# MP-Gadget/shenqi

Hardware: AMD Instinct MI355X
Metric: particle-steps/sec (grav+PM+SPH) at 256^3; rms force error vs ref (higher is better)
Workload: dtype f64

## Files before the change

__graft_entry__.py:

```python
import os
import subprocess
import sys

ROOT = os.path.dirname(os.path.abspath(__file__))


def build():
    env = dict(os.environ)
    env.setdefault("HIPCC", "/opt/rocm/bin/hipcc")
    subprocess.check_call(["make", "-C", ROOT, "-j4", "all"], env=env)
    if ROOT not in sys.path:
        sys.path.insert(0, ROOT)
    import shenqi_amd


def smoke():
    if ROOT not in sys.path:
        sys.path.insert(0, ROOT)
    sys.path.insert(0, os.path.join(ROOT, "tests"))
    import numpy as np
    import shenqi_amd as sq
    import common as cm
    import orc

    n = 16**3
    pos = cm.random_positions(orc.boost_mt19937_uniform(0, 3 * n), n)
    pman = cm.make_partmanager(pos)
    pm = dict(Asmth=1.5, Nmesh=48, G=cm.G)
    cm.reference_treepar(ErrTolForceAcc=0.002, MaxBHOpeningAngle=0.9, TreeUseBH=0)
    sq.gravshort_set_softenings(cm.BOX / np.cbrt(n))
    gp_rel = sq.make_grav_params(cm.BOX, 1.5, 48, cm.G, cm.RHO0)
    with sq.Context(0) as ctx:
        sq.gravpm_force(ctx, pm, pman)
        tree = sq.force_tree_full(pman)
        cm.reference_treepar(ErrTolForceAcc=0.002, MaxBHOpeningAngle=0.9)
        sq.gravshort_set_softenings(cm.BOX / np.cbrt(n))
        sq.grav_short_tree(ctx, None, pm, tree, None, cm.RHO0)
        gpm = pman.Base["GravPM"].copy()
        seed = pman.Base["FullTreeGravAccel"].copy()
        st = sq.grav_short_tree(ctx, None, pm, tree, None, cm.RHO0)
        acc = pman.Base["FullTreeGravAccel"].copy()
        import ctypes as C
        from shenqi_amd import capi
        tb = sq.tree_build_device(ctx, cm.BOX)
        capi.check(capi.hip.shq_grav_short_run(ctx.h, C.byref(gp_rel), None, 0, 1, sq.WALK_EXACT))
        nint_dev = np.zeros(n, dtype=np.int64)
        capi.check(capi.hip.shq_grav_short_download(ctx.h, None, None, capi.ptr(nint_dev), None))
        pmp = sq.PMParams(48, 0, cm.BOX, 1.5, cm.G)
        capi.check(capi.hip.shq_treepm_step(ctx.h, C.byref(pmp), C.byref(gp_rel), 1, sq.WALK_EXACT))
        fused = C.c_int(0)
        capi.check(capi.hip.shq_treepm_last_fused(ctx.h, C.byref(fused)))
        gpm_step = np.zeros((n, 3)); acc_step = np.zeros((n, 3)); nint_step = np.zeros(n, dtype=np.int64)
        capi.check(capi.hip.shq_pm_download(ctx.h, capi.ptr(gpm_step), None))
        capi.check(capi.hip.shq_grav_short_download(ctx.h, capi.ptr(acc_step), None, capi.ptr(nint_step), None))
    mass = pman.Base["Mass"]
    ogpm, _, _, _ = orc.pm_force(pos, mass, 48, cm.BOX, 1.5, cm.G)
    cm.reference_treepar(ErrTolForceAcc=0.002, MaxBHOpeningAngle=0.9, TreeUseBH=0)
    gp = sq.make_grav_params(cm.BOX, 1.5, 48, cm.G, cm.RHO0)
    oacc, opot, onint = orc.grav_walk(tree.Nodes_base, tree.firstnode, pos, mass,
                                      np.linalg.norm(seed + gpm, axis=1) / cm.G, gp)
    oacc *= cm.G
    e_pm = np.abs(gpm - ogpm).max() / np.abs(ogpm).max()
    e_tree = np.abs(acc - oacc).max() / np.abs(oacc).max()
    assert e_pm < 1e-9, e_pm
    assert e_tree < 1e-10, e_tree
    assert st.ninteractions == int(onint.sum())
    assert tb.numnodes > 0 and np.array_equal(nint_dev, onint), "walk on the device-built tree differs from the oracle"
    assert fused.value == 0, "shq_treepm_step took the fused-readout route, which is off by default"
    assert np.abs(gpm_step - ogpm).max() / np.abs(ogpm).max() < 1e-9
    oacc2, _, onint2 = orc.grav_walk(tree.Nodes_base, tree.firstnode, pos, mass, np.linalg.norm(acc + gpm_step, axis=1) / cm.G, gp)
    assert np.array_equal(nint_step, onint2), "shq_treepm_step: interaction counts differ from the oracle"
    assert np.abs(acc_step - oacc2 * cm.G).max() / np.abs(oacc2).max() / cm.G < 1e-10
    ng = 10**3
    gpos = cm.BOX * orc.boost_mt19937_uniform(7, 3 * ng).reshape(ng, 3)
    gman, SphP, BhP = cm.make_gas(gpos, np.full(ng, cm.BOX / 10))
    BhP = np.zeros(2, dtype=sq.BH_SLOT_DTYPE)
    sq.set_densitypar(DensityResolutionEta=1.0, MaxNumNgbDeviation=0.5, DensityKernelType=1, BlackHoleNgbFactor=2.0, MinGasHsml=0.006)
    ost = orc.SphState(gman.Base, SphP, BhP)
    onodes, ofirst, ofather = orc.tree_build(gpos, gman.Base["Mass"], cm.BOX)
    rc, oevp, _, oniter, _ = orc.density(onodes, ofirst, ofather, ost, cm.density_params(DoEgyDensity=1))
    assert rc == 0
    orc.update_hmax(onodes, ofirst, ost)
    orc.hydro(onodes, ofirst, ost, cm.hydro_params(), oevp)
    with sq.Context(0) as ctx:
        gtree = sq.force_tree_rebuild_mask(gman, sq.GASMASK)
        evp, dst = sq.density(ctx, None, 1, 1, 0, None, gtree, gman, SphP, BhP)
        sq.force_tree_update_hmax(gtree, gman)
        sq.set_hydropar(1, 100.0, 0.75)
        sq.hydro_force(ctx, None, 0.1, cm.HUBBLE, evp, None, gtree, gman, SphP)
    e_rho = np.abs(SphP["Density"] / ost.density - 1).max()
    e_hyd = np.abs(SphP["HydroAccel"] - ost.hydroaccel).max() / np.abs(ost.hydroaccel).max()
    assert dst.niterations == oniter and e_rho < 1e-10 and e_hyd < 1e-9, (dst.niterations, oniter, e_rho, e_hyd)
    print(f"smoke ok: PM rel err {e_pm:.2e}, tree rel err {e_tree:.2e}, SPH density rel err {e_rho:.2e}, hydro rel err {e_hyd:.2e}, "
          f"{st.ninteractions / n:.1f} interactions/target, walk {st.kernel_ms:.3f} ms, "
          f"device tree build {tb.numnodes} nodes in {tb.build_ms:.3f} ms")


if __name__ == "__main__":
    build()
    if len(sys.argv) > 1 and sys.argv[1] == "smoke":
        smoke()
```

shenqi_amd/csrc/common.hpp:

```cpp
#ifndef SHQ_COMMON_HPP
#define SHQ_COMMON_HPP

#include <hip/hip_runtime.h>
#include <hipfft/hipfft.h>
#include <stdint.h>
#include <stdio.h>
#include <string>
#include <vector>
#include "../../include/shenqi_hip.h"
#include "yields_math.hpp"
#include "cooling_math.hpp"

void shq_set_error(const char *fmt, ...);

#define SHQ_HIP(call)                                                                          \
    do {                                                                                       \
        hipError_t e_ = (call);                                                                \
        if(e_ != hipSuccess) {                                                                 \
            shq_set_error("%s:%d: %s failed: %s", __FILE__, __LINE__, #call, hipGetErrorString(e_)); \
            return (e_ == hipErrorOutOfMemory) ? SHQ_ERR_NOMEM : SHQ_ERR_DEVICE;               \
        }                                                                                      \
    } while(0)

#define SHQ_CHECK(cond, code, ...)                                                             \
// ... 30 lines not shown
            ptr = nullptr;
            return SHQ_ERR_NOMEM;
        }
        cap = n;
        return SHQ_OK;
    }
    void release()
    {
        if(ptr)
            (void) hipFree(ptr);
        ptr = nullptr;
        cap = 0;
    }
};

template <typename T> struct PinBuf {
    T *ptr = nullptr;
    size_t cap = 0;
    int reserve(size_t n)
    {
        if(n <= cap)
            return SHQ_OK;
        if(ptr)
            (void) hipHostFree(ptr);
        ptr = nullptr;
        cap = 0;
        hipError_t e = hipHostMalloc((void **) &ptr, n * sizeof(T), hipHostMallocDefault);
        if(e != hipSuccess) {
            shq_set_error("hipHostMalloc of %zu bytes failed: %s", n * sizeof(T), hipGetErrorString(e));
            ptr = nullptr;
            return SHQ_ERR_NOMEM;
        }
        cap = n;
        return SHQ_OK;
    }
    void release()
    {
        if(ptr)
            (void) hipHostFree(ptr);
        ptr = nullptr;
        cap = 0;
    }
};

struct NodeA { double cofm[3]; double mass; };
struct NodeB { double center[3]; double len; };
struct NodeC { int32_t sibling; int32_t child; int32_t type; int32_t count; };
struct NodeH { double hmax; };
struct alignas(128) NodeG {
    double cofm[3], mass;
    double center[3], len;
    int32_t sibling, child, type, count;
    double bhlim;
    double mlen2;
    double inside;
    double rcut2;
    double wraplim;
    double rcuthl;
};
static_assert(sizeof(NodeG) == 128, "NodeG must be one 128-byte line");

struct alignas(32) TopNodeG {
    double cofm[3], mass;
    double center[3], len;
    double hmax;
    int32_t sibling, child;
    int32_t kind;
    int32_t leaf;
    double pad;
};
static_assert(sizeof(TopNodeG) == 96, "TopNodeG layout");

struct GravStatsDev {
    unsigned long long ninteractions;
    unsigned long long nvisited;
    unsigned long long nwave_applies;
    unsigned long long nwave_node_applies;
    unsigned long long nnode_interactions;
    long long min_int;
    long long max_int;
    unsigned long long hist_visit[8], hist_node[8], hist_leaf[8];
    unsigned long long lonely[4];
};

__device__ __forceinline__ unsigned long long shq_ballot(bool p) { return __builtin_amdgcn_ballot_w64(p); }

__device__ __forceinline__ unsigned xcd_block(unsigned b, unsigned nb, unsigned K = 16)
{
    if(K == 0)
        return b;
    const unsigned super = b / (8u * K);
    if((super + 1u) * 8u * K > nb)
        return b;
    const unsigned within = b - super * 8u * K;
    return super * 8u * K + (within & 7u) * K + (within >> 3);
}

#define SHQ_NTIMERS 20
enum { SHQ_T_PM0 = 8 , SHQ_T_SPH = 14, SHQ_T_TREE = 16, SHQ_T_WALK = SHQ_NTIMERS - 1 };

struct TreeBuildBufs {
    DevBuf<unsigned long long> keys[2], okeys[2], packed[2], counters;
    DevBuf<int> state;
    DevBuf<int32_t> idx[2], order[2], rank, frontier[2], bounds;
    DevBuf<int32_t> lo, hi, parent, sibling, firstchild, nchild, level;
    DevBuf<int32_t> top;
    DevBuf<unsigned long long> path;
    DevBuf<int4> geo_child[2];
    DevBuf<int2> geo_kind;
    DevBuf<double> topbuf;
    DevBuf<double4> cen, mom;
    DevBuf<double> hmax;
    DevBuf<shq_node> exportbuf;
    void release()
    {
        for(int i = 0; i < 2; i++) {
            keys[i].release(); okeys[i].release(); packed[i].release(); idx[i].release(); order[i].release(); frontier[i].release();
        }
        counters.release(); rank.release(); bounds.release(); lo.release(); hi.release(); parent.release(); sibling.release();
        firstchild.release(); nchild.release(); level.release(); cen.release(); mom.release(); hmax.release();
        exportbuf.release(); top.release(); path.release(); geo_child[0].release(); geo_child[1].release(); geo_kind.release(); topbuf.release(); state.release();
    }
};

struct shq_fft_plan {
    int N = 0;
    struct {
        unsigned res_z = 0, res_s = 0, res_x = 0, res_x3 = 0, res_x4 = 0, res_x5 = 0;
    } t;
    struct {
        unsigned res_zf = 0, res_zi = 0, res_s = 0, res_x3 = 0, res_x4 = 0;
    } n;
};

struct shq_context {
    int device = 0;
    hipStream_t stream = nullptr;
    bool own_stream = false;
    hipStream_t stream_walk = nullptr;
    hipEvent_t ev_walk_in = nullptr, ev_walk_out = nullptr;
    hipStream_t stream_pm = nullptr;
    hipEvent_t ev_pm_ready = nullptr, ev_pm_done = nullptr;
    hipStream_t stream_pair = nullptr;
    hipEvent_t ev_pair_fork = nullptr, ev_pair_join = nullptr;
    int inputs_current = 0;
    const void *cur_parts = nullptr, *cur_sph = nullptr, *cur_tree = nullptr, *cur_ids = nullptr;
    int64_t cur_parts_n = -1, cur_sph_n = -1, cur_tree_n = -1, cur_tree_first = -1, cur_ids_n = -1;
    hipEvent_t ev_sph[4] = {nullptr, nullptr, nullptr, nullptr};
    bool pm_pending = false;
    bool pm_prestarted = false;
    bool pm_prestarted_oldacc = false;
    int pm_prestarted_nmesh = 0;
    bool pm_overlap = false;
    bool treepm_fuse = false;
    double readout_oldacc_G = 0;
    bool last_step_fused = false;
    bool fuse_readout = false;
    double fuse_cell = 0, fuse_ffac = 0, fuse_G = 0;
    DevBuf<double> mesh_alt;
    bool pm_scrub = true;
    bool mesh_zeroed = false;
    size_t mesh_words = 0;
    hipEvent_t ev_begin[SHQ_NTIMERS] = {};
    hipEvent_t ev_end[SHQ_NTIMERS] = {};

    int64_t numpart = 0;
    int64_t nlocal = 0;
    DevBuf<double4> posm;
    DevBuf<double> oldacc;
    DevBuf<double> treeacc;
    DevBuf<double> gravpm;
    DevBuf<double> pmpot;
    DevBuf<double> acc;
    DevBuf<double> pot;
    DevBuf<int32_t> nint;
    DevBuf<uint8_t> pflags;
    DevBuf<int32_t> active;
    DevBuf<unsigned long long> top_task;
    DevBuf<int32_t> top_sort;
    DevBuf<long long> top_slot;
    long long top_ntargets = 0, top_nexport = -1;
    DevBuf<TopNodeG> topnodes;
    DevBuf<int2> topleaves;
    DevBuf<int32_t> top_counts;
    DevBuf<shq_data_index> top_table;
    int64_t ntopnodes = 0;
    bool tb_domain = false;
    std::vector<shq_topnode_geo> dom_geo;
    std::vector<int32_t> dom_kind, dom_rank, dom_leaf_task;
    std::vector<double> dom_rec;
    int dom_thistask = 0;
    bool have_toptree = false;
    bool grav_raw = false;
    DevBuf<shq_grav_result> gq_res;
    DevBuf<int32_t> act_list, act_sub;
    DevBuf<unsigned long long> act_counts;
    DevBuf<uint8_t> act_flag;
    int64_t n_act = -1, n_sub = -1;
    bool act_all = false;
    DevBuf<GravStatsDev> gstats;
    DevBuf<char> prim_temp;
    bool have_parts = false;
    int stats_guard = 0;
    bool allow_padding = false;

    int64_t numnodes = 0;
    int64_t firstnode = 0;
    int32_t root = 0;
    int64_t ntreeparts = 0;
    DevBuf<NodeA> nodeA;
    DevBuf<NodeB> nodeB;
    DevBuf<NodeC> nodeC;
    DevBuf<NodeG> nodeG;
    DevBuf<double4> posm_leaf;
    DevBuf<int32_t> leaf_pidx;
    bool have_tree = false;
    DevBuf<float4> nodeF;
    bool have_group_aux = false;
    DevBuf<int> walk_counters;
    DevBuf<int32_t> walk_pool_idx, walk_chunk_cnt, walk_chunk_next, walk_group_head;
    DevBuf<uint8_t> walk_pool_msk;
    int64_t walk_pool_chunks = 0;
    double walk_chunks_per_target = 0;
    double node_rcut = -1;
    double node_bh2 = -1;
    double treeBox = 0;
    DevBuf<double> node_hmax;
    DevBuf<int32_t> pfather;
    DevBuf<int32_t> node_father;
    std::vector<int32_t> node_order;
    std::vector<int32_t> node_rank;
    bool have_father = false;
    TreeBuildBufs tb;
    int64_t tb_initial_cap = 0;
    int tb_attempts = 0;
    DevBuf<int32_t> tree_targets;
    int64_t ntree_targets = 0;
    bool have_tree_targets = false;
    int tree_targets_refresh = 8;
    int tree_targets_age = 0, tree_targets_mask = -2;
    long long tree_targets_np = -1, tree_targets_ntree = -1;
    DevBuf<int32_t> bhw_bhp, bhw_queue;
    DevBuf<char> bhw_rec;
    DevBuf<unsigned long long> bhw_ids, bhw_sphsw, bhw_bhsw, bhw_swid;
    DevBuf<double> bhw_rnd, bhw_out;
    DevBuf<uint8_t> bhw_eeqos, bhw_heated, bhw_touched;
    DevBuf<int32_t> bhw_tlist;
    DevBuf<double> bhw_trows;
    DevBuf<unsigned long long> metal_keys[2];
    DevBuf<double> metal_val[2], metal_star, metal_gd;
    DevBuf<float> metal_gf;
    DevBuf<char> wind_kicks;
    DevBuf<double> wind_d;
    DevBuf<unsigned long long> wind_cnt;
    bool tb_built = false;

    bool have_sph = false;
    bool have_dyn = false;
    DevBuf<double> hsml, dthsml, vel;
    DevBuf<uint8_t> bin_grav, bin_hydro;
    DevBuf<double> g_entropy, g_dtentropy, g_hydroaccel, g_delaytime;
    DevBuf<double> g_density, g_egywt, g_dhsmlegy, g_divvel, g_curlvel;
    DevBuf<double> g_hydroaccel_out, g_dtentropy_out, g_maxsignalvel;
    bool gas_resident = false;
    DevBuf<int> gas_bad;
    DevBuf<int32_t> ex_list, ex_val[3];
    DevBuf<unsigned int> ex_key[4];
    DevBuf<unsigned long long> ex_counts, ex_u64;
    DevBuf<long long> ex_i64;
    DevBuf<char> ex_bytes;
    std::vector<shq_exchange_entry> ex_togo;
    int64_t ex_last = -1;
    int ex_ntask = 0;
    DevBuf<uint16_t> dd_tab;
    shq_peano_tables dd_tab_src = {};
    bool dd_tab_valid = false;
    DevBuf<char> dd_nodes;
    DevBuf<int32_t> dd_leaf_task;
    int dd_ntopnodes = 0, dd_ntopleaves = 0;
    DevBuf<unsigned long long> dd_u64[3];
    DevBuf<long long> dd_i64[2];
    DevBuf<int32_t> dd_i32[3];
    DevBuf<uint8_t> dd_u8;
    DevBuf<char> dd_rec;
    DevBuf<uint8_t> io_u8[2];
    DevBuf<unsigned long long> io_u64[2];
    DevBuf<int32_t> io_i32;
    DevBuf<unsigned long long> io_cnt;
    DevBuf<long long> st_cnt;
    DevBuf<double> st_part, st_old;
    DevBuf<int32_t> st_i32;
    DevBuf<unsigned long long> stat_cnt;
    DevBuf<double> stat_part;
    DevBuf<uint8_t> stat_mark;
    DevBuf<int32_t> stat_list, stat_pos;
    DevBuf<double> lc_reps;
    DevBuf<int32_t> lc_cnt;
    DevBuf<long long> lc_off;
    double lc_ms[3] = {0, 0, 0};
    DevBuf<int32_t> fof_parent, fof_i32[6], fof_g32[5], fof_partgrnr, fof_members, fof_biglist;
    DevBuf<unsigned long long> fof_u64[4];
    DevBuf<unsigned int> fof_gkey[2];
    DevBuf<long long> fof_goff[2];
    DevBuf<shq_fof_group> fof_groups;
    DevBuf<char> fof_partial;
    int64_t fof_ngroups = -1, fof_nmembers = 0, fof_nruns = 0;
    bool have_bh_dyn = false, bh_reposition = false;
// ... 360 lines not shown
```

shenqi_amd/csrc/grav_walk.hip:

```cpp
#include "common.hpp"
#include "pm_readout.hpp"
#include <utility>
#include <stdlib.h>

namespace {

struct WalkArgs {
    const NodeG *nodeG;
    const double4 *posm;
    const double4 *posm_leaf;
    const double *oldacc;
    const int32_t *targets;
    const int32_t *qstart;
    double *acc;
    double *pot;
    int32_t *nint;
    GravStatsDev *stats;
    long long ntargets;
    int root;
    double Box, invBox, halfBox;
    double rcut, rcut2;
    double h, h2, h_inv, h3_inv;
    double inv_celldx;
    double errtol, bh2;
// ... 75 lines not shown
    }
    const double fi = fmin(r * a.inv_celldx, (double) (SHQ_NGRAVTAB - 1));
    const int ti = (int) fi;
    const double w1 = __builtin_amdgcn_fract(fi);
    if(POT) {
        const double4 t = tab[ti];
        fac *= fma(w1, t.y, t.x);
        pot = fma(-npot, fma(w1, t.w, t.z), pot);
    } else {
        const double2 t = *reinterpret_cast<const double2 *>(&tab[ti]);
        fac *= fma(w1, t.y, t.x);
    }
    ax = fma(dx, fac, ax);
    ay = fma(dy, fac, ay);
    az = fma(dz, fac, az);
}

template <bool POT>
__device__ __forceinline__ void leaf_particle(const double4 *__restrict__ tab, const double4 q, double px, double py,
                                              double pz, const WalkArgs &a, double &ax, double &ay, double &az,
                                              double &pot, const unsigned long long wrapm)
{
    double ex = q.x - px, ey = q.y - py, ez = q.z - pz;
    if(wrapm != 0ull) {
        ex = wrapd(ex, a.Box, a.invBox);
        ey = wrapd(ey, a.Box, a.invBox);
        ez = wrapd(ez, a.Box, a.invBox);
    }
    const double rr2 = ex * ex + ey * ey + ez * ez;
    apply_accn<POT>(tab, ex, ey, ez, rr2, q.w, a, ax, ay, az, pot);
}

#if defined(__HIP_DEVICE_COMPILE__)
#define SHQ_CONSTANT_AS __attribute__((address_space(4)))
#else
#define SHQ_CONSTANT_AS
#endif
typedef const SHQ_CONSTANT_AS WalkArgs *WalkArgsK;
__device__ __forceinline__ WalkArgsK walk_cold_args()
{
    WalkArgsK kp = (WalkArgsK) __builtin_amdgcn_kernarg_segment_ptr();
    asm volatile("" : "+s"(kp));
    return kp;
}

template <typename T> __device__ __forceinline__ void agent_store(T *p, T v) { __hip_atomic_store(p, v, __ATOMIC_RELAXED, __HIP_MEMORY_SCOPE_AGENT); }
template <typename T> __device__ __forceinline__ T agent_load(const T *p) { return __hip_atomic_load(const_cast<T *>(p), __ATOMIC_RELAXED, __HIP_MEMORY_SCOPE_AGENT); }

__device__ __forceinline__ int walk_next_task(WalkArgsK c, int &region, int &tried)
{
    const int lg = c->task_run_log2;
    const int nwaves = (int) c->nwaves;
    unsigned int *counters = c->task_counters;
    while(tried < 8) {
        unsigned k = 0;
        if((threadIdx.x & 63) == 0)
            k = atomicAdd(&counters[16 * region], 1u);
        k = (unsigned) __builtin_amdgcn_readfirstlane((int) k);
        const unsigned t = ((((k >> lg) << 3) + (unsigned) region) << lg) | (k & ((1u << lg) - 1u));
        if(k < 0x40000000u && t < (unsigned) nwaves)
            return (int) t;
        region = (region + 1) & 7;
        tried++;
    }
    return -1;
}

#define SHQ_LEAF_RING 32
#ifndef SHQ_SPARSE_LANES
#define SHQ_SPARSE_LANES 8
#endif
#ifndef SHQ_SPARSE_CAP
#define SHQ_SPARSE_CAP 96
#endif
#define SHQ_SPARSE_STACK 4096
#define SHQ_SPARSE_SPIN (1u << 22)
#ifndef SHQ_PAIR_DEPTH2
#define SHQ_PAIR_DEPTH2 1
#endif
enum SpFlag {
    SP_OVERFLOW = 0,
    SP_GAVEUP = 1,
    SP_MOPPED = 2,
    SP_HIGHWATER = 3,
    SP_STICKY_ERROR = 8,
    SP_STICKY_RECOVERED = 9,
    SP_STICKY_HIGHWATER = 10,
    SP_TASK_COUNTER = 16
};
#define SP_TASK_DONE (-2)
#ifndef SHQ_PAIR_WAVES
#define SHQ_PAIR_WAVES 8
#define SHQ_PAIR_WG_PER_CU 2
#define SHQ_PAIR_EU 4
#endif

template <bool POT>
__device__ __forceinline__ void leaf_ring_drain(const double4 *__restrict__ tab, const double4 *ring, unsigned &mymask, double px, double py,
                                                double pz, const WalkArgs &a, double &ax, double &ay, double &az, double &pot,
                                                const unsigned long long wrapm)
{
    asm volatile("s_waitcnt vmcnt(0)" ::: "memory");
    while(shq_ballot(mymask != 0u) != 0ull) {
        if(mymask != 0u) {
            const int b = __builtin_ctz(mymask);
            mymask &= mymask - 1u;
            const double4 q = ring[b];
            leaf_particle<POT>(tab, q, px, py, pz, a, ax, ay, az, pot, wrapm);
        }
    }
}

template <bool POT, bool PREFETCH, int LEAFB, int STATS, bool BH, bool GHOSTS = false, bool PERSIST = false, bool RING = false, bool READOUT = false,
          bool SPARSE = false>
__global__ __launch_bounds__(512) __attribute__((amdgpu_num_sgpr(96), amdgpu_num_vgpr(64))) void grav_walk_exact_kernel(const WalkArgs a)
{
    extern __shared__ double4 ring_all[];
    double4 *const ring = ring_all + (threadIdx.x >> 6) * SHQ_LEAF_RING;
    __shared__ double4 tab[SHQ_NGRAVTAB];
    for(int i = threadIdx.x; i < SHQ_NGRAVTAB; i += blockDim.x) {
        const int j = (i + 1 < SHQ_NGRAVTAB) ? i + 1 : i;
        const double f0 = a.tab_f[i], f1 = a.tab_f[j], p0 = a.tab_p[i], p1 = a.tab_p[j];
        tab[i] = i + 1 < SHQ_NGRAVTAB ? make_double4(f0, f1 - f0, p0, p1 - p0) : make_double4(0, 0, 0, 0);
    }
    __syncthreads();

    typedef const SHQ_CONSTANT_AS NodeG *NodeGK;
    typedef const SHQ_CONSTANT_AS double4 *Double4K;
    const NodeGK nodeG = (NodeGK) (size_t) a.nodeG;
    const Double4K posm_leaf = (Double4K) (size_t) a.posm_leaf;
    const int lane = threadIdx.x & 63;
    int region = blockIdx.x & 7, tried = 0;
    long long wave = PERSIST ? (long long) walk_next_task(walk_cold_args(), region, tried)
                             : (long long) xcd_block(blockIdx.x, gridDim.x, a.xcdK) * (blockDim.x >> 6) + (threadIdx.x >> 6);
    while(wave >= 0) {
    const long long t = wave * 64 + lane;
    long long pi = 0;
    double px = 0, py = 0, pz = 0, aold = 0;
    bool valid;
    {
        const WalkArgs c = PERSIST ? *walk_cold_args() : a;
        valid = t < c.ntargets;
        if(valid) {
            pi = c.targets ? (long long) c.targets[t] : t;
            valid = pi >= 0;
        }
        if(valid) {
            const double4 p = c.posm[pi];
            px = p.x;
            py = p.y;
            pz = p.z;
            if(READOUT) {
                double g0 = 0, g1 = 0, g2 = 0, gp = 0;
                pm_readout_lean(c.pm_mesh, c.pmN, c.pmzp, c.pmcell, c.pmffac, px, py, pz, !(c.pflags && (c.pflags[pi] & 2)), g0, g1, g2, gp);
                c.gravpm[3 * pi + 0] = g0;
                c.gravpm[3 * pi + 1] = g1;
                c.gravpm[3 * pi + 2] = g2;
                c.pmpot[pi] = gp;
                const double gv[3] = {g0, g1, g2};
                double s = 0;
                {
#pragma clang fp contract(off)
                    for(int j = 0; j < 3; j++) {
                        const double ax = c.treeacc[3 * pi + j] + gv[j];
                        s += ax * ax;
                    }
                }
                const double oa = sqrt(s) / c.G;
                if(SPARSE)
                    agent_store(&c.oldacc_out[pi], oa);
                else
                    c.oldacc_out[pi] = oa;
                aold = c.errtol * oa;
            } else
                aold = c.errtol * c.oldacc[pi];
        }
        if(c.scrub_per_task > 0) {
            const long long u0 = wave * c.scrub_per_task + lane;
            for(int k = 0; k < c.scrub_per_task; k += 64)
                if(u0 + k < c.scrub_n16) {
                    unsigned z = 0;
                    asm volatile("" : "+v"(z));
                    c.scrub[u0 + k] = make_uint4(z, z, z, z);
                }
        }
    }
    double ax = 0, ay = 0, az = 0, pot = 0;
    int nint = 0;
    int sp_n = 0;
    unsigned ringmask = 0;
    int ringfill = 0;
    unsigned long long ringwrap = 0;
    unsigned int node_int_wave = 0;
    int mynext = valid ? a.root : -2;
    int cur = a.root;
    int seg1 = -1, seg2 = -1, seg3 = -1, myend = -1;
    if(GHOSTS) {
        mynext = -2;
        if(valid) {
            const int4 st = *reinterpret_cast<const int4 *>(a.qstart + 4 * t);
            mynext = st.x >= 0 ? st.x : -2;
            seg1 = st.y; seg2 = st.z; seg3 = st.w;
            if(mynext >= 0)
                myend = a.nodeG[mynext].sibling;
        }
    }
    unsigned int visited = 0, wave_applies = 0, wave_node_applies = 0;
    unsigned int hv[8] = {}, hn[8] = {}, hl[8] = {};
    unsigned int lonely8 = 0, lonely16 = 0;

    do {
        const NodeG nd = nodeG[cur];
        if(STATS)
            visited++;
        const bool act = (mynext == cur);
        if(STATS == 2)
            hv[(__popcll(shq_ballot(mynext == cur)) - 1) >> 3 & 7]++;

        double dx = nd.cofm[0] - px, dy = nd.cofm[1] - py, dz = nd.cofm[2] - pz;
        double ux = nd.center[0] - px, uy = nd.center[1] - py, uz = nd.center[2] - pz;
        double cmax = fmax(fmax(fabs(ux), fabs(uy)), fabs(uz));
        const unsigned long long actm = shq_ballot(mynext == cur);
        unsigned long long wrapm = 0ull;
        int wl_hi = __double2hiint(nd.wraplim);
        asm volatile("" : "+s"(wl_hi));
        if(wl_hi >= 0) {
            asm volatile("" ::: "memory");
            wrapm = shq_ballot(cmax >= nd.wraplim) & actm;
            if(wrapm != 0ull) {
                dx = wrapd(dx, a.Box, a.invBox);
                dy = wrapd(dy, a.Box, a.invBox);
                dz = wrapd(dz, a.Box, a.invBox);
                ux = wrapd(ux, a.Box, a.invBox);
                uy = wrapd(uy, a.Box, a.invBox);
                uz = wrapd(uz, a.Box, a.invBox);
                cmax = fmax(fmax(fabs(ux), fabs(uy)), fabs(uz));
            }
        }
        const double r2 = dx * dx + dy * dy + dz * dz;
        const unsigned long long keepm = actm & ~(shq_ballot(r2 > nd.rcut2) & shq_ballot(cmax > nd.rcuthl));
        const unsigned long long openm = (BH ? 0ull : shq_ballot(nd.mlen2 > r2 * r2 * aold)) | shq_ballot(r2 < nd.bhlim) |
                                         shq_ballot(cmax < nd.inside);
        const unsigned long long acceptm = keepm & ~openm, doopenm = keepm & openm;
        const bool accept = __builtin_amdgcn_inverse_ballot_w64(acceptm), doopen = __builtin_amdgcn_inverse_ballot_w64(doopenm);

        {
            if(STATS && acceptm != 0ull) {
                wave_applies++;
                wave_node_applies++;
                node_int_wave += (unsigned int) __popcll(acceptm);
            }
            if(STATS == 2 && acceptm != 0ull) {
                const int pc = __popcll(acceptm);
                hn[(pc - 1) >> 3 & 7]++;
                if(accept && pc <= 8)
                    lonely8++;
                if(accept && pc <= 16)
                    lonely16++;
            }
            if(accept) {
                apply_accn<POT, false>(tab, dx, dy, dz, r2, nd.mass, a, ax, ay, az, pot);
                nint++;
            }
        }
        int next;
        if(nd.type == SHQ_PARTICLE_NODE_TYPE) {
            asm volatile("" ::: "memory");
            if(RING && doopenm != 0ull) {
                const int cnt = nd.count;
                if(ringfill + cnt > SHQ_LEAF_RING) {
                    leaf_ring_drain<POT>(tab, ring, ringmask, px, py, pz, a, ax, ay, az, pot, ringwrap);
                    ringfill = 0;
                    ringwrap = 0;
                }
                if(lane < 2 * cnt)
                    __builtin_amdgcn_global_load_lds(reinterpret_cast<const double2 *>(a.posm_leaf + nd.child) + lane,
                                                     (__attribute__((address_space(3))) void *) (ring + ringfill), 16, 0, 0);
                if(doopen) {
                    ringmask |= ((1u << cnt) - 1u) << ringfill;
                    nint += cnt;
                }
                ringfill += cnt;
                ringwrap |= wrapm;
            }
            if(!RING && doopenm != 0ull) {
                const Double4K lp = posm_leaf + nd.child;
                const int cnt = nd.count;
                if(STATS)
                    wave_applies += cnt;
                if(STATS == 2) {
                    const int pc = __popcll(doopenm);
                    hl[(pc - 1) >> 3 & 7] += cnt;
                    if(doopen && pc <= 8)
                        lonely8 += cnt;
                    if(doopen && pc <= 16)
                        lonely16 += cnt;
                }
#pragma unroll
                for(int b = 0; b < SHQ_NMAXCHILD; b += LEAFB) {
                    if(b < cnt) {
                        double4 q[LEAFB];
#pragma unroll
                        for(int k = 0; k < LEAFB; k++)
                            q[k] = lp[b + k];
                        if(doopen) {
#pragma unroll
                            for(int k = 0; k < LEAFB; k++)
// ... 1041 lines not shown
```

shenqi_amd/csrc/pm.hip:

```cpp
#include "mesh_common.hpp"
#include "pm_readout.hpp"
#include <math.h>
#include <stdlib.h>
#include <string.h>

namespace {

static unsigned pm_xcdk(int deposit)
{
    static const unsigned kr = getenv("SHQ_PM_XCD_K") ? (unsigned) atoi(getenv("SHQ_PM_XCD_K")) : 64u;
    static const unsigned kd = getenv("SHQ_PM_DEP_XCD_K") ? (unsigned) atoi(getenv("SHQ_PM_DEP_XCD_K")) : 0u;
    return deposit ? kd : kr;
}

__global__ void pm_zero_kernel(unsigned long long *mesh, size_t n)
{
    size_t i = (size_t) blockIdx.x * blockDim.x + threadIdx.x;
    const size_t stride = (size_t) gridDim.x * blockDim.x;
    for(; i < n; i += stride)
        mesh[i] = 0ull;
}

#ifndef DEP_T
#define DEP_T 16
// ... 23 lines not shown
    bool ok[DEP_PPT];
    int lmin[3] = {0x7fffffff, 0x7fffffff, 0x7fffffff}, lmax[3] = {-0x7fffffff, -0x7fffffff, -0x7fffffff};
#pragma unroll
    for(int j = 0; j < DEP_PPT; j++) {
        const long long i = base + (long long) j * 256 + tid;
        ok[j] = (i < n) && !(pflags && ((pflags[i] & 2) || !((typemask >> (pflags[i] >> 4)) & 1u)));
        mass[j] = 0;
        if(ok[j]) {
            const double4 p = posm[i];
            cic_setup(p.x, cell, N, ic[j][0], res[j][0]);
            cic_setup(p.y, cell, N, ic[j][1], res[j][1]);
            cic_setup(p.z, cell, N, ic[j][2], res[j][2]);
            mass[j] = p.w;
#pragma unroll
            for(int k = 0; k < 3; k++) {
                lmin[k] = min(lmin[k], ic[j][k]);
                lmax[k] = max(lmax[k], ic[j][k]);
            }
        }
    }
#pragma unroll
    for(int k = 0; k < 3; k++) {
        int mn = lmin[k], mx = lmax[k];
        for(int off = 32; off > 0; off >>= 1) {
            mn = min(mn, __shfl_xor(mn, off));
            mx = max(mx, __shfl_xor(mx, off));
        }
        if((tid & 63) == 0) {
            atomicMin(&s_min[k], mn);
            atomicMax(&s_max[k], mx);
        }
    }
    __syncthreads();
    const int m0 = s_min[0], m1 = s_min[1], m2 = s_min[2];
    const bool fits = (s_max[0] - m0 + 2 <= DEP_T) && (s_max[1] - m1 + 2 <= DEP_T) && (s_max[2] - m2 + 2 <= DEP_T);
    const size_t sy = (size_t) zp, sx = (size_t) N * zp;
    if(fits) {
        const int ey = s_max[1] - m1 + 2, ez = s_max[2] - m2 + 2, vol = (s_max[0] - m0 + 2) * ey * ez;
        for(int c = tid; c < vol; c += 256)
            tile[c] = 0ull;
        __syncthreads();
#pragma unroll
        for(int j = 0; j < DEP_PPT; j++) {
            if(!ok[j])
                continue;
#pragma unroll
            for(int c = 0; c < 8; c++) {
                double w = 1.0;
                int lin = 0;
#pragma unroll
                for(int k = 0; k < 3; k++) {
                    const int off = (c >> k) & 1;
                    const int t = ic[j][k] - (k == 0 ? m0 : (k == 1 ? m1 : m2)) + off;
                    lin = lin * (k == 0 ? 1 : (k == 1 ? ey : ez)) + t;
                    w *= off ? res[j][k] : (1 - res[j][k]);
                }
                const long long q = __double2ll_rn(w * mass[j] * scale);
                atomicAdd(&tile[lin], (unsigned long long) q);
            }
        }
        __syncthreads();
        for(int c = tid; c < vol; c += 256) {
            const unsigned long long v = tile[c];
            if(v != 0ull) {
                const int tz = c % ez, ty = (c / ez) % ey, tx = c / (ez * ey);
                const int lx = xloc(m0 + tx, xshift, N);
                if(lx >= nxalloc) {
                    *oob = 1;
                    continue;
                }
                const size_t lin = (size_t) lx * sx + (size_t) wrapi(m1 + ty, N) * sy + (size_t) wrapi(m2 + tz, N);
                atomicAdd(&mesh[lin], v);
            }
        }
    } else {
        static_assert(DEP_T * DEP_T * DEP_T >= 4 * 8 * 64 * 2, "the staging area is the LDS tile");
        ulonglong2 *const stg = reinterpret_cast<ulonglong2 *>(tile) + (tid >> 6) * (8 * 64);
        const int lane = tid & 63;
#pragma unroll
        for(int j = 0; j < DEP_PPT; j++) {
#pragma unroll
            for(int c = 0; c < 8; c++) {
                double w = 1.0;
                size_t lin = 0;
                bool inb = true;
#pragma unroll
                for(int k = 0; k < 3; k++) {
                    const int off = (c >> k) & 1;
                    const int t = (k == 0) ? xloc(ic[j][k] + off, xshift, N) : wrapi(ic[j][k] + off, N);
                    if(k == 0 && t >= nxalloc)
                        inb = false;
                    lin += (size_t) t * (k == 0 ? sx : (k == 1 ? sy : 1));
                    w *= off ? res[j][k] : (1 - res[j][k]);
                }
                const long long q = __double2ll_rn(w * mass[j] * scale);
                if(ok[j] && !inb)
                    *oob = 1;
                stg[((c & 3) * 2 + (c >> 2)) * 64 + lane] = make_ulonglong2(ok[j] && inb ? (unsigned long long) lin : ~0ull, (unsigned long long) q);
            }
            __builtin_amdgcn_fence(__ATOMIC_RELEASE, "wavefront");
            __builtin_amdgcn_wave_barrier();
            __builtin_amdgcn_fence(__ATOMIC_ACQUIRE, "wavefront");
#pragma unroll
            for(int k = 0; k < 8; k++) {
                const ulonglong2 e = stg[((k & 3) * 2 + (lane & 1)) * 64 + (lane >> 1) + 32 * (k >> 2)];
                if(e.x != ~0ull)
                    atomicAdd(&mesh[e.x], e.y);
            }
            __builtin_amdgcn_fence(__ATOMIC_RELEASE, "wavefront");
            __builtin_amdgcn_wave_barrier();
            __builtin_amdgcn_fence(__ATOMIC_ACQUIRE, "wavefront");
        }
    }
}

__global__ __launch_bounds__(256) void pm_green_kernel(double2 *cmesh, int N, int Nc, int zpc, const double *__restrict__ sinctab,
                                                       double asmth2, double pot_factor, const double *__restrict__ T = nullptr)
{
    const size_t total = (size_t) N * N * Nc;
    size_t ip = (size_t) blockIdx.x * blockDim.x + threadIdx.x;
    if(ip >= total)
        return;
    const int z = (int) (ip % Nc);
    const size_t xy = ip / Nc;
    ip = xy * (size_t) zpc + z;
    const int y = (int) (xy % N);
    const int x = (int) (xy / N);
    const int kx = x <= N / 2 ? x : x - N;
    const int ky = y <= N / 2 ? y : y - N;
    const int kz = z;
    const long long k2 = (long long) kx * kx + (long long) ky * ky + (long long) kz * kz;
    double2 v = cmesh[ip];
    if(k2 == 0) {
        v.x = 0;
        v.y = 0;
    } else {
        if(T) {
            const double t = T[k2];
            v.x *= t;
            v.y *= t;
        }
        double f = 1.0;
        const double smth = exp(-(double) k2 * asmth2) / (double) k2;
        f *= sinctab[x];
        f *= sinctab[y];
        f *= sinctab[z];
        const double fac = pot_factor * smth * f * f;
        v.x *= fac;
        v.y *= fac;
    }
    cmesh[ip] = v;
}

struct __attribute__((aligned(8))) pair8 { double x, y; };

__global__ __launch_bounds__(256) void pm_readout_kernel(const double4 *__restrict__ posm, const uint8_t *__restrict__ pflags,
                                                         long long n, const double *__restrict__ mesh, int N, int zp,
                                                         double cell, double ffac, double *gravpm, double *pmpot, int xshift,
                                                         int nxalloc, int *oob, unsigned xcdk, const double *__restrict__ treeacc = nullptr,
                                                         double *oldacc = nullptr, double G = 0)
{
#pragma clang fp contract(off)
    const long long i = (long long) xcd_block(blockIdx.x, gridDim.x, xcdk) * blockDim.x + threadIdx.x;
    if(i >= n)
        return;
    double g0 = 0, g1 = 0, g2 = 0, gp = 0;
    if(!(pflags && (pflags[i] & 2))) {
        const double4 p = posm[i];
        int ic[3];
        double res[3];
        cic_setup(p.x, cell, N, ic[0], res[0]);
        cic_setup(p.y, cell, N, ic[1], res[1]);
        cic_setup(p.z, cell, N, ic[2], res[2]);
        const size_t sy = (size_t) zp, sx = (size_t) N * zp;
        size_t ox[6], oy[6], oz[6];
#pragma unroll
        for(int d = 0; d < 6; d++) {
            const int lx = xloc(ic[0] + d - 2, xshift, N);
            if(lx >= nxalloc && oob)
                *oob = 1;
            ox[d] = (size_t) (lx < nxalloc ? lx : 0) * sx;
            oy[d] = (size_t) wrapi(ic[1] + d - 2, N) * sy;
            oz[d] = (size_t) wrapi(ic[2] + d - 2, N);
        }
        const double c1 = 2.0 / 3.0, c2 = 1.0 / 12.0;
        if(ic[2] >= 2 && ic[2] + 3 < N) {
            const double *m = mesh + (ic[2] - 2);
            pair8 xl[2][6], yl[2][6], zl[2][2][3];
#pragma unroll
            for(int b2 = 0; b2 < 2; b2++)
#pragma unroll
                for(int d = 0; d < 6; d++)
                    xl[b2][d] = *reinterpret_cast<const pair8 *>(m + ox[d] + oy[2 + b2] + 2);
#pragma unroll
            for(int a2 = 0; a2 < 2; a2++)
#pragma unroll
                for(int d = 0; d < 6; d++)
                    yl[a2][d] = (d == 2 || d == 3) ? xl[d - 2][2 + a2] : *reinterpret_cast<const pair8 *>(m + ox[2 + a2] + oy[d] + 2);
#pragma unroll
            for(int a2 = 0; a2 < 2; a2++)
#pragma unroll
                for(int b2 = 0; b2 < 2; b2++) {
                    zl[a2][b2][0] = *reinterpret_cast<const pair8 *>(m + ox[2 + a2] + oy[2 + b2]);
                    zl[a2][b2][1] = xl[b2][2 + a2];
                    zl[a2][b2][2] = *reinterpret_cast<const pair8 *>(m + ox[2 + a2] + oy[2 + b2] + 4);
                }
#pragma unroll
            for(int c = 0; c < 8; c++) {
                const int a = c & 1, b = (c >> 1) & 1, e = (c >> 2) & 1;
                const double w = (a ? res[0] : 1 - res[0]) * (b ? res[1] : 1 - res[1]) * (e ? res[2] : 1 - res[2]);
                const int X = 2 + a, Y = 2 + b, Z = 2 + e;
#define PZ(P) ((e) ? (P).y : (P).x)
#define ZV(K) (((K) & 1) ? zl[a][b][(K) >> 1].y : zl[a][b][(K) >> 1].x)
                const double phi = PZ(xl[b][X]);
                const double fx = ffac * (c1 * (PZ(xl[b][X + 1]) - PZ(xl[b][X - 1])) - c2 * (PZ(xl[b][X + 2]) - PZ(xl[b][X - 2])));
                const double fy = ffac * (c1 * (PZ(yl[a][Y + 1]) - PZ(yl[a][Y - 1])) - c2 * (PZ(yl[a][Y + 2]) - PZ(yl[a][Y - 2])));
                const double fz = ffac * (c1 * (ZV(Z + 1) - ZV(Z - 1)) - c2 * (ZV(Z + 2) - ZV(Z - 2)));
#undef PZ
#undef ZV
                gp += w * phi;
                g0 += w * fx;
                g1 += w * fy;
                g2 += w * fz;
            }
        } else {
            auto M = [&](int dx, int dy, int dz) { return mesh[ox[2 + dx] + oy[2 + dy] + oz[2 + dz]]; };
#pragma unroll
            for(int c = 0; c < 8; c++)
                pm_readout_corner<0>(c, res, ffac, M, g0, g1, g2, gp);
        }
    }
    gravpm[3 * i + 0] = g0;
    gravpm[3 * i + 1] = g1;
    gravpm[3 * i + 2] = g2;
    pmpot[i] = gp;
    if(oldacc) {
        const double gv[3] = {g0, g1, g2};
        double s = 0;
        for(int j = 0; j < 3; j++) {
            const double ax = treeacc[3 * i + j] + gv[j];
            s += ax * ax;
        }
        oldacc[i] = sqrt(s) / G;
    }
}

__global__ void pm_repitch_kernel(const double *src, double *dst, size_t nrows, int len, int spitch, int dpitch, int as_i64,
                                  double inv_scale)
{
    const size_t total = nrows * (size_t) len;
    size_t ip = (size_t) blockIdx.x * blockDim.x + threadIdx.x;
    if(ip >= total)
        return;
    const int z = (int) (ip % len);
    const size_t row = ip / len;
    if(as_i64)
        dst[row * dpitch + z] = (double) reinterpret_cast<const long long *>(src)[row * spitch + z] * inv_scale;
    else
        dst[row * dpitch + z] = src[row * spitch + z];
}

}

void shq_pm_destroy_plans(shq_context *ctx)
{
    if(ctx->have_plans) {
        hipfftDestroy(ctx->plan_r2c);
        hipfftDestroy(ctx->plan_c2r);
        ctx->have_plans = false;
    }
    ctx->pm_nmesh = 0;
    ctx->pm_custom_fft = false;
}

static int pm_prepare(shq_context *ctx, int N)
{
    SHQ_CHECK(N >= 4 && N % 2 == 0, SHQ_ERR_INVALID, "Nmesh must be even and >= 4 (got %d)", N);
    ctx->mesh_zeroed = false;
    if(ctx->pm_nmesh == N && (ctx->have_plans || ctx->pm_custom_fft))
        return SHQ_OK;
    shq_pm_destroy_plans(ctx);
    ctx->pm_custom_fft = shq_fft3d_supported(N) && !getenv("SHQ_PM_ROCFFT");
    ctx->pm_zp = ctx->pm_custom_fft ? shq_fft3d_pitch(N) : N + 2;
    const size_t padded = (size_t) N * N * ctx->pm_zp;
    SHQ_TRY(ctx->mesh.reserve(padded));
    ctx->mesh_words = padded;
    SHQ_TRY(ctx->sinctab.reserve(N));
    SHQ_TRY(ctx->pm_oob.reserve(1));
    SHQ_HIP(hipMemset(ctx->pm_oob.ptr, 0, sizeof(int)));
    std::vector<double> tab(N);
    for(int i = 0; i < N; i++) {
        const int k = i <= N / 2 ? i : i - N;
        double tmp = (k * M_PI) / N;
        double s;
        if(tmp < 1e-5 && tmp > -1e-5) {
            double x2 = tmp * tmp;
            s = 1.0 - x2 / 6. + x2 * x2 / 120.;
        } else
            s = sin(tmp) / tmp;
        tab[i] = 1. / (s * s);
    }
    SHQ_HIP(hipMemcpy(ctx->sinctab.ptr, tab.data(), sizeof(double) * N, hipMemcpyHostToDevice));
    ctx->sinctab_n = N;
    ctx->pm_nmesh = N;
    if(ctx->pm_custom_fft)
        return SHQ_OK;
    hipfftResult r = hipfftPlan3d(&ctx->plan_r2c, N, N, N, HIPFFT_D2Z);
    SHQ_CHECK(r == HIPFFT_SUCCESS, SHQ_ERR_DEVICE, "hipfftPlan3d(D2Z, %d) failed: %d", N, (int) r);
    r = hipfftPlan3d(&ctx->plan_c2r, N, N, N, HIPFFT_Z2D);
    SHQ_CHECK(r == HIPFFT_SUCCESS, SHQ_ERR_DEVICE, "hipfftPlan3d(Z2D, %d) failed: %d", N, (int) r);
    hipfftSetStream(ctx->plan_r2c, ctx->stream);
    hipfftSetStream(ctx->plan_c2r, ctx->stream);
    ctx->have_plans = true;
    ctx->pm_nmesh = N;
    return SHQ_OK;
}

namespace {

__device__ __forceinline__ void pm_power_add(double *hist, int nbins, int N, const int32_t *__restrict__ bintab, const double *__restrict__ sinctab,
                                             double *norm, double2 v, int x, int y, int kz, long long k2)
{
    const double m = v.x * v.x + v.y * v.y;
    if(k2 == 0) {
        *norm = m;
        return;
    }
    const int kint = bintab[k2];
    if(kint >= nbins)
        return;
    const double f = sinctab[x] * sinctab[y] * sinctab[kz];
    const double w = (kz == 0 || kz == N / 2) ? 1.0 : 2.0;
    atomicAdd(&hist[kint], w * m * f * f);
    atomicAdd(&hist[nbins + kint], w * sqrt((double) k2));
    atomicAdd(&hist[2 * nbins + kint], w);
}

__device__ __forceinline__ void pm_power_flush(const double *hist, int nbins, double *power, double *kk, unsigned long long *nmodes)
{
    __syncthreads();
    for(int i = threadIdx.x; i < nbins; i += blockDim.x) {
        if(hist[2 * nbins + i] != 0) {
            atomicAdd(&power[i], hist[i]);
            atomicAdd(&kk[i], hist[nbins + i]);
            atomicAdd(&nmodes[i], (unsigned long long) hist[2 * nbins + i]);
        }
    }
}

__global__ __launch_bounds__(256) void pm_power_kernel(const double2 *__restrict__ cmesh, int N, int Nc, int zpc, const double *__restrict__ sinctab,
                                                       const int32_t *__restrict__ bintab, int nbins, double *power, double *kk,
                                                       unsigned long long *nmodes, double *norm, const double *__restrict__ T = nullptr,
                                                       int nzb = 0)
{
    extern __shared__ double hist[];
    for(int i = threadIdx.x; i < 3 * nbins; i += blockDim.x)
        hist[i] = 0;
    __syncthreads();
    const size_t total = nzb > 0 ? (size_t) N * nzb * N * 4 : (size_t) N * N * Nc;
    for(size_t ip = (size_t) blockIdx.x * blockDim.x + threadIdx.x; ip < total; ip += (size_t) gridDim.x * blockDim.x) {
        int x, y, z;
        size_t at;
        if(nzb > 0) {
            const size_t r = (ip >> 2) / N;
            x = (int) ((ip >> 2) % N);
            y = (int) (r / nzb);
            z = 4 * (int) (r % nzb) + (int) (ip & 3);
            at = ip;
            if(z >= Nc)
                continue;
        } else {
            z = (int) (ip % Nc);
// ... 910 lines not shown
```

shenqi_amd/csrc/pm_readout.hpp:

```cpp
#pragma once
#include "cic.hpp"
#ifndef SHQ_READOUT_FENCE
#define SHQ_READOUT_FENCE 1
#endif

template <int FENCE, typename MeshAt>
__device__ __forceinline__ void pm_readout_corner(int c, const double res[3], double ffac, MeshAt M, double &g0, double &g1, double &g2,
                                                  double &gp)
{
#pragma clang fp contract(off)
    const double c1 = 2.0 / 3.0, c2 = 1.0 / 12.0;
    const int a = c & 1, b = (c >> 1) & 1, e = (c >> 2) & 1;
    auto side = [](int bit, double r) { return fma(bit ? 1.0 : -1.0, r, bit ? 0.0 : 1.0); };
    const double w = side(a, res[0]) * side(b, res[1]) * side(e, res[2]);
#define SHQ_PM_DIFF(P1, M1, P2, M2)                                \
    [&]() {                                                        \
        double d1 = (P1) - (M1);                                   \
        if(FENCE == 1)                                             \
            asm volatile("" : "+v"(d1)::"memory");                 \
        double d2 = (P2) - (M2);                                   \
        if(FENCE)                                                  \
            asm volatile("" : "+v"(d1), "+v"(d2)::"memory");       \
        return ffac * (c1 * d1 - c2 * d2);                         \
    }()
    double phi = M(a, b, e);
    if(FENCE == 1)
        asm volatile("" : "+v"(phi)::"memory");
    const double fz = SHQ_PM_DIFF(M(a, b, e + 1), M(a, b, e - 1), M(a, b, e + 2), M(a, b, e - 2));
    const double fx = SHQ_PM_DIFF(M(a + 1, b, e), M(a - 1, b, e), M(a + 2, b, e), M(a - 2, b, e));
    const double fy = SHQ_PM_DIFF(M(a, b + 1, e), M(a, b - 1, e), M(a, b + 2, e), M(a, b - 2, e));
#undef SHQ_PM_DIFF
    gp += w * phi;
    g0 += w * fx;
    g1 += w * fy;
    g2 += w * fz;
    if(FENCE)
        asm volatile("" : "+v"(g0), "+v"(g1), "+v"(g2), "+v"(gp)::"memory");
}

__device__ __forceinline__ void pm_readout_lean(const double *__restrict__ mesh, int N, int zp, double cell, double ffac, double px, double py,
                                                double pz, bool live, double &g0, double &g1, double &g2, double &gp)
{
    int ic[3];
    double res[3];
    cic_setup(px, cell, N, ic[0], res[0]);
    cic_setup(py, cell, N, ic[1], res[1]);
    cic_setup(pz, cell, N, ic[2], res[2]);
    g0 = g1 = g2 = gp = 0;
    const unsigned sy = (unsigned) zp, sx = (unsigned) N * (unsigned) zp;
    const bool inner = ic[0] >= 2 && ic[0] + 3 < N && ic[1] >= 2 && ic[1] + 3 < N && ic[2] >= 2 && ic[2] + 3 < N;
    const bool interior = __builtin_amdgcn_ballot_w64(live && !inner) == 0ull;
    if(interior) {
        if(live) {
            const unsigned vb = (((unsigned) ic[0] * sx + (unsigned) ic[1] * sy + (unsigned) ic[2]) << 3);
            const char *base = reinterpret_cast<const char *>(mesh);
#pragma unroll
            for(int c = 0; c < 8; c++) {
                long long sxc = (long long) sx * 8, syc = (long long) sy * 8;
                asm volatile("" : "+s"(sxc), "+s"(syc));
                auto M = [&](int dx, int dy, int dz) {
                    typedef const __attribute__((address_space(1))) char *GlobalBytes;
                    GlobalBytes sb = (GlobalBytes) (base + (dx * sxc + dy * syc + dz * 8));
                    asm volatile("" : "+s"(sb));
                    return *reinterpret_cast<const __attribute__((address_space(1))) double *>(sb + vb);
                };
                pm_readout_corner<SHQ_READOUT_FENCE>(c, res, ffac, M, g0, g1, g2, gp);
            }
        }
    } else if(live) {
#pragma unroll 1
        for(int c = 0; c < 8; c++) {
            auto M = [&](int dx, int dy, int dz) {
                const unsigned o = (unsigned) wrapi(ic[0] + dx, N) * sx + (unsigned) wrapi(ic[1] + dy, N) * sy + (unsigned) wrapi(ic[2] + dz, N);
                return *reinterpret_cast<const double *>(reinterpret_cast<const char *>(mesh) + (o << 3));
            };
            pm_readout_corner<1>(c, res, ffac, M, g0, g1, g2, gp);
        }
    }
}
```

Baseline: 419.3 million.

## Enable fused PM readout in tree walk by default with paired-load readout

Turns on the fused TreePM path by default, so the PM force readout runs inside the gravity walk kernel instead of as a separate readout pass. The interior readout now fetches mesh values as 16-byte pairs along z, reusing them across corners and grouping loads by axis, instead of issuing scalar loads per corner. The intent is to cut the separate kernel launch, its mesh traffic and the number of load instructions. In exchange the walk kernel gets more register pressure, and the summation order has to stay bit-compatible, which is why fences and contract(off) are kept.

```diff
diff --git a/__graft_entry__.py b/__graft_entry__.py
--- a/__graft_entry__.py
+++ b/__graft_entry__.py
@@ -66,7 +66,7 @@
     assert e_tree < 1e-10, e_tree
     assert st.ninteractions == int(onint.sum())
     assert tb.numnodes > 0 and np.array_equal(nint_dev, onint), "walk on the device-built tree differs from the oracle"
-    assert fused.value == 0, "shq_treepm_step took the fused-readout route, which is off by default"
+    assert fused.value == 1, "shq_treepm_step did not take the fused-readout route, which is the default"
     assert np.abs(gpm_step - ogpm).max() / np.abs(ogpm).max() < 1e-9
     oacc2, _, onint2 = orc.grav_walk(tree.Nodes_base, tree.firstnode, pos, mass, np.linalg.norm(acc + gpm_step, axis=1) / cm.G, gp)
     assert np.array_equal(nint_step, onint2), "shq_treepm_step: interaction counts differ from the oracle"
diff --git a/shenqi_amd/csrc/common.hpp b/shenqi_amd/csrc/common.hpp
--- a/shenqi_amd/csrc/common.hpp
+++ b/shenqi_amd/csrc/common.hpp
@@ -206,7 +206,7 @@
     bool pm_prestarted_oldacc = false;
     int pm_prestarted_nmesh = 0;
     bool pm_overlap = false;
-    bool treepm_fuse = false;
+    bool treepm_fuse = true;
     double readout_oldacc_G = 0;
     bool last_step_fused = false;
     bool fuse_readout = false;
diff --git a/shenqi_amd/csrc/grav_walk.hip b/shenqi_amd/csrc/grav_walk.hip
--- a/shenqi_amd/csrc/grav_walk.hip
+++ b/shenqi_amd/csrc/grav_walk.hip
@@ -251,7 +251,7 @@
             pz = p.z;
             if(READOUT) {
                 double g0 = 0, g1 = 0, g2 = 0, gp = 0;
-                pm_readout_lean(c.pm_mesh, c.pmN, c.pmzp, c.pmcell, c.pmffac, px, py, pz, !(c.pflags && (c.pflags[pi] & 2)), g0, g1, g2, gp);
+                pm_readout_lean<SHQ_READOUT_PAIRS>(c.pm_mesh, c.pmN, c.pmzp, c.pmcell, c.pmffac, px, py, pz, !(c.pflags && (c.pflags[pi] & 2)), g0, g1, g2, gp);
                 c.gravpm[3 * pi + 0] = g0;
                 c.gravpm[3 * pi + 1] = g1;
                 c.gravpm[3 * pi + 2] = g2;
diff --git a/shenqi_amd/csrc/pm.hip b/shenqi_amd/csrc/pm.hip
--- a/shenqi_amd/csrc/pm.hip
+++ b/shenqi_amd/csrc/pm.hip
@@ -199,8 +199,6 @@
     cmesh[ip] = v;
 }
 
-struct __attribute__((aligned(8))) pair8 { double x, y; };
-
 __global__ __launch_bounds__(256) void pm_readout_kernel(const double4 *__restrict__ posm, const uint8_t *__restrict__ pflags,
                                                          long long n, const double *__restrict__ mesh, int N, int zp,
                                                          double cell, double ffac, double *gravpm, double *pmpot, int xshift,
@@ -230,41 +228,35 @@
             oy[d] = (size_t) wrapi(ic[1] + d - 2, N) * sy;
             oz[d] = (size_t) wrapi(ic[2] + d - 2, N);
         }
-        const double c1 = 2.0 / 3.0, c2 = 1.0 / 12.0;
         if(ic[2] >= 2 && ic[2] + 3 < N) {
-            const double *m = mesh + (ic[2] - 2);
+            auto P = [&](PmPair p) { return *reinterpret_cast<const pair8 *>(mesh + ox[2 + p.dx] + oy[2 + p.dy] + (ic[2] + p.dz)); };
             pair8 xl[2][6], yl[2][6], zl[2][2][3];
 #pragma unroll
             for(int b2 = 0; b2 < 2; b2++)
 #pragma unroll
                 for(int d = 0; d < 6; d++)
-                    xl[b2][d] = *reinterpret_cast<const pair8 *>(m + ox[d] + oy[2 + b2] + 2);
+                    xl[b2][d] = P(pm_pair_x(b2, d));
 #pragma unroll
             for(int a2 = 0; a2 < 2; a2++)
 #pragma unroll
                 for(int d = 0; d < 6; d++)
-                    yl[a2][d] = (d == 2 || d == 3) ? xl[d - 2][2 + a2] : *reinterpret_cast<const pair8 *>(m + ox[2 + a2] + oy[d] + 2);
+                    yl[a2][d] = (d == 2 || d == 3) ? xl[d - 2][2 + a2] : P(pm_pair_y(a2, d));
 #pragma unroll
             for(int a2 = 0; a2 < 2; a2++)
 #pragma unroll
                 for(int b2 = 0; b2 < 2; b2++) {
-                    zl[a2][b2][0] = *reinterpret_cast<const pair8 *>(m + ox[2 + a2] + oy[2 + b2]);
+                    zl[a2][b2][0] = P(pm_pair_z(a2, b2, 0));
                     zl[a2][b2][1] = xl[b2][2 + a2];
-                    zl[a2][b2][2] = *reinterpret_cast<const pair8 *>(m + ox[2 + a2] + oy[2 + b2] + 4);
+                    zl[a2][b2][2] = P(pm_pair_z(a2, b2, 2));
                 }
 #pragma unroll
             for(int c = 0; c < 8; c++) {
                 const int a = c & 1, b = (c >> 1) & 1, e = (c >> 2) & 1;
-                const double w = (a ? res[0] : 1 - res[0]) * (b ? res[1] : 1 - res[1]) * (e ? res[2] : 1 - res[2]);
-                const int X = 2 + a, Y = 2 + b, Z = 2 + e;
-#define PZ(P) ((e) ? (P).y : (P).x)
-#define ZV(K) (((K) & 1) ? zl[a][b][(K) >> 1].y : zl[a][b][(K) >> 1].x)
-                const double phi = PZ(xl[b][X]);
-                const double fx = ffac * (c1 * (PZ(xl[b][X + 1]) - PZ(xl[b][X - 1])) - c2 * (PZ(xl[b][X + 2]) - PZ(xl[b][X - 2])));
-                const double fy = ffac * (c1 * (PZ(yl[a][Y + 1]) - PZ(yl[a][Y - 1])) - c2 * (PZ(yl[a][Y + 2]) - PZ(yl[a][Y - 2])));
-                const double fz = ffac * (c1 * (ZV(Z + 1) - ZV(Z - 1)) - c2 * (ZV(Z + 2) - ZV(Z - 2)));
-#undef PZ
-#undef ZV
+                const double w = pm_pair_weight(c, res);
+                const double phi = pm_pair_el(xl[b][2 + a], e);
+                const double fx = pm_pair_force(xl[b], 2 + a, e, ffac);
+                const double fy = pm_pair_force(yl[a], 2 + b, e, ffac);
+                const double fz = pm_pair_force_z(zl[a][b], e, ffac);
                 gp += w * phi;
                 g0 += w * fx;
                 g1 += w * fy;
diff --git a/shenqi_amd/csrc/pm_readout.hpp b/shenqi_amd/csrc/pm_readout.hpp
--- a/shenqi_amd/csrc/pm_readout.hpp
+++ b/shenqi_amd/csrc/pm_readout.hpp
@@ -1,9 +1,5 @@
 #pragma once
 #include "cic.hpp"
-#ifndef SHQ_READOUT_FENCE
-#define SHQ_READOUT_FENCE 1
-#endif
-
 template <int FENCE, typename MeshAt>
 __device__ __forceinline__ void pm_readout_corner(int c, const double res[3], double ffac, MeshAt M, double &g0, double &g1, double &g2,
                                                   double &gp)
@@ -38,6 +34,66 @@
         asm volatile("" : "+v"(g0), "+v"(g1), "+v"(g2), "+v"(gp)::"memory");
 }
 
+struct __attribute__((aligned(8))) pair8 { double x, y; };
+struct PmPair { int dx, dy, dz; };
+__host__ __device__ constexpr PmPair pm_pair_x(int b, int d) { return PmPair{d - 2, b, 0}; }
+__host__ __device__ constexpr PmPair pm_pair_y(int a, int d) { return PmPair{a, d - 2, 0}; }
+__host__ __device__ constexpr PmPair pm_pair_z(int a, int b, int k) { return PmPair{a, b, 2 * k - 2}; }
+
+__device__ __forceinline__ double pm_pair_el(const pair8 &p, int e) { return e ? p.y : p.x; }
+__device__ __forceinline__ double pm_pair_weight(int c, const double res[3])
+{
+#pragma clang fp contract(off)
+    const int a = c & 1, b = (c >> 1) & 1, e = (c >> 2) & 1;
+    return (a ? res[0] : 1 - res[0]) * (b ? res[1] : 1 - res[1]) * (e ? res[2] : 1 - res[2]);
+}
+__device__ __forceinline__ double pm_pair_force(const pair8 *l, int X, int e, double ffac)
+{
+#pragma clang fp contract(off)
+    const double c1 = 2.0 / 3.0, c2 = 1.0 / 12.0;
+    return ffac * (c1 * (pm_pair_el(l[X + 1], e) - pm_pair_el(l[X - 1], e)) - c2 * (pm_pair_el(l[X + 2], e) - pm_pair_el(l[X - 2], e)));
+}
+__device__ __forceinline__ double pm_pair_force_z(const pair8 *z, int e, double ffac)
+{
+#pragma clang fp contract(off)
+    const double c1 = 2.0 / 3.0, c2 = 1.0 / 12.0;
+    auto zv = [&](int k) { return pm_pair_el(z[k >> 1], k & 1); };
+    const int Z = 2 + e;
+    return ffac * (c1 * (zv(Z + 1) - zv(Z - 1)) - c2 * (zv(Z + 2) - zv(Z - 2)));
+}
+
+#ifndef SHQ_READOUT_PAIRS
+#define SHQ_READOUT_PAIRS 4
+#endif
+
+template <int PIF, int NP, typename PairOf>
+__device__ __forceinline__ void pm_fetch_pairs(pair8 *l, const char *base, unsigned vb, unsigned sx, unsigned sy, PairOf pairof)
+{
+#if defined(__HIP_DEVICE_COMPILE__)
+#define SHQ_GLOBAL_AS __attribute__((address_space(1)))
+#else
+#define SHQ_GLOBAL_AS
+#endif
+    typedef const SHQ_GLOBAL_AS char *GlobalBytes;
+    long long sxc = (long long) sx * 8, syc = (long long) sy * 8;
+    asm volatile("" : "+s"(sxc), "+s"(syc));
+#pragma unroll
+    for(int k0 = 0; k0 < NP; k0 += PIF) {
+#pragma unroll
+        for(int k = k0; k < k0 + PIF && k < NP; k++) {
+            const PmPair p = pairof(k);
+            GlobalBytes sb = (GlobalBytes) (base + (p.dx * sxc + p.dy * syc));
+            asm volatile("" : "+s"(sb));
+            l[k] = *reinterpret_cast<const SHQ_GLOBAL_AS pair8 *>(sb + vb + p.dz * 8);
+        }
+#pragma unroll
+        for(int k = k0; k < k0 + PIF && k < NP; k++)
+            asm volatile("" : "+v"(l[k].x), "+v"(l[k].y)::"memory");
+    }
+#undef SHQ_GLOBAL_AS
+}
+
+template <int PIF>
 __device__ __forceinline__ void pm_readout_lean(const double *__restrict__ mesh, int N, int zp, double cell, double ffac, double px, double py,
                                                 double pz, bool live, double &g0, double &g1, double &g2, double &gp)
 {
@@ -52,20 +108,84 @@
     const bool interior = __builtin_amdgcn_ballot_w64(live && !inner) == 0ull;
     if(interior) {
         if(live) {
+#pragma clang fp contract(off)
             const unsigned vb = (((unsigned) ic[0] * sx + (unsigned) ic[1] * sy + (unsigned) ic[2]) << 3);
             const char *base = reinterpret_cast<const char *>(mesh);
-#pragma unroll
-            for(int c = 0; c < 8; c++) {
-                long long sxc = (long long) sx * 8, syc = (long long) sy * 8;
-                asm volatile("" : "+s"(sxc), "+s"(syc));
-                auto M = [&](int dx, int dy, int dz) {
-                    typedef const __attribute__((address_space(1))) char *GlobalBytes;
-                    GlobalBytes sb = (GlobalBytes) (base + (dx * sxc + dy * syc + dz * 8));
-                    asm volatile("" : "+s"(sb));
-                    return *reinterpret_cast<const __attribute__((address_space(1))) double *>(sb + vb);
-                };
-                pm_readout_corner<SHQ_READOUT_FENCE>(c, res, ffac, M, g0, g1, g2, gp);
-            }
+#define SHQ_PM_UNIT_DONE(V) asm volatile("" : "+v"(V[0][0]), "+v"(V[0][1]), "+v"(V[1][0]), "+v"(V[1][1]), "+v"(res[0]), "+v"(res[1]), "+v"(res[2]))
+            double hp[4], hz[4], hx[2], hy[2][2];
+#pragma unroll
+            for(int c = 0; c < 4; c++) {
+                pair8 l[3];
+                double v[2][2];
+                pm_fetch_pairs<PIF, 3>(l, base, vb, sx, sy, [c](int k) { return pm_pair_z(c & 1, c >> 1, k); });
+#pragma unroll
+                for(int e = 0; e < 2; e++) {
+                    v[0][e] = pm_pair_el(l[1], e);
+                    v[1][e] = pm_pair_force_z(l, e, ffac);
+                }
+                SHQ_PM_UNIT_DONE(v);
+                const double w = pm_pair_weight(c, res);
+                gp += w * v[0][0];
+                g2 += w * v[1][0];
+                hp[c] = v[0][1];
+                hz[c] = v[1][1];
+                asm volatile("" : "+v"(gp), "+v"(g2), "+v"(hp[c]), "+v"(hz[c])::"memory");
+            }
+#pragma unroll
+            for(int c = 4; c < 8; c++) {
+                const double w = pm_pair_weight(c, res);
+                gp += w * hp[c - 4];
+                g2 += w * hz[c - 4];
+            }
+            asm volatile("" : "+v"(gp), "+v"(g2)::"memory");
+#pragma unroll
+            for(int b = 0; b < 2; b++) {
+                pair8 l[6];
+                double f[2][2];
+                pm_fetch_pairs<PIF, 6>(l, base, vb, sx, sy, [b](int k) { return pm_pair_x(b, k); });
+#pragma unroll
+                for(int a = 0; a < 2; a++)
+#pragma unroll
+                    for(int e = 0; e < 2; e++)
+                        f[a][e] = pm_pair_force(l, 2 + a, e, ffac);
+                SHQ_PM_UNIT_DONE(f);
+#pragma unroll
+                for(int a = 0; a < 2; a++)
+                    g0 += pm_pair_weight(a + 2 * b, res) * f[a][0];
+#pragma unroll
+                for(int c = 4; c < 8; c++) {
+                    if(b == 0 && c < 6)
+                        hx[c & 1] = f[c & 1][1];
+                    if(b == 1)
+                        g0 += pm_pair_weight(c, res) * (c < 6 ? hx[c & 1] : f[c & 1][1]);
+                }
+                asm volatile("" : "+v"(g0), "+v"(hx[0]), "+v"(hx[1])::"memory");
+            }
+#pragma unroll
+            for(int a = 0; a < 2; a++) {
+                pair8 l[6];
+                double f[2][2];
+                pm_fetch_pairs<PIF, 6>(l, base, vb, sx, sy, [a](int k) { return pm_pair_y(a, k); });
+#pragma unroll
+                for(int b = 0; b < 2; b++)
+#pragma unroll
+                    for(int e = 0; e < 2; e++)
+                        f[b][e] = pm_pair_force(l, 2 + b, e, ffac);
+                SHQ_PM_UNIT_DONE(f);
+#pragma unroll
+                for(int c = 0; c < 8; c++) {
+                    const int b = (c >> 1) & 1, e = (c >> 2) & 1;
+                    if(a == 0 && c == 0)
+                        g1 += pm_pair_weight(c, res) * f[b][e];
+                    if(a == 0 && c > 0 && !(c & 1))
+                        hy[b][e] = f[b][e];
+                    if(a == 1 && c > 0)
+                        g1 += pm_pair_weight(c, res) * ((c & 1) ? f[b][e] : hy[b][e]);
+                }
+                if(a == 0)
+                    asm volatile("" : "+v"(g1), "+v"(hy[1][0]), "+v"(hy[0][1]), "+v"(hy[1][1])::"memory");
+            }
+#undef SHQ_PM_UNIT_DONE
         }
     } else if(live) {
 #pragma unroll 1
```

New measurement: 434.0 million, median of 6. 1.03x the previous value.
